# Hjinhan/Transgo

Measured on AMD Instinct MI355X. Metric: MCTS simulations/sec, higher is better.
Workload: dtype f32

## Files before the change

### include/transgo_hip.h

```cpp
#ifndef TRANSGO_HIP_H_
#define TRANSGO_HIP_H_

#include <stdbool.h>
#include <stddef.h>
#include <stdint.h>

#ifdef __cplusplus
extern "C" {
#endif

typedef struct tg_ctx tg_ctx;

typedef enum tg_status {
    TG_OK = 0,
    TG_ERR_ARG = -1,
    TG_ERR_HIP = -2,
    TG_ERR_NO_DEVICE = -3,
    TG_ERR_ARENA = -4,
    TG_ERR_STATE = -5
} tg_status;

typedef struct tg_config {
    int32_t board_size;
    int32_t encode_dim;
// ... 56 lines not shown

int tg_sp_collect(tg_ctx* ctx, int32_t* n_active, int32_t* n_rows);
int tg_sp_absorb(tg_ctx* ctx);
int tg_sp_search(tg_ctx* ctx, int32_t* n_waves);

int tg_sp_root_info(tg_ctx* ctx, int32_t* visits , int32_t* root_n, int32_t* player, int32_t* step,
                    float* obs );
int tg_sp_draw_uniform(tg_ctx* ctx, double* u , const uint8_t* mask);
int tg_sp_rng_state(tg_ctx* ctx, int game, tg_mt19937* out);
int tg_sp_rng_get(tg_ctx* ctx, tg_mt19937* out );
int tg_sp_rng_set(tg_ctx* ctx, const tg_mt19937* in , const uint8_t* mask );
int tg_sp_play(tg_ctx* ctx, const int32_t* actions , uint8_t* done );
int tg_sp_game_errors(tg_ctx* ctx, int32_t* n_errors, int32_t* err );
int tg_sp_tree_truncations(tg_ctx* ctx, uint64_t* blocks);

int tg_sp_pool_stats(tg_ctx* ctx, uint64_t* pool_slots, uint64_t* high_water_slots, uint64_t* in_use_slots, uint64_t* exhausted);

int tg_sp_finished(tg_ctx* ctx, int32_t* n_games, int32_t* n_positions);
int tg_sp_harvest(tg_ctx* ctx, uint32_t* obs_bits, int32_t* counts, float* z, int8_t* own, uint8_t* player, int device_out,
                  int32_t* slot, int32_t* n_moves, int32_t* winner, float* score, int8_t* terr);
int tg_sp_final(tg_ctx* ctx, float* score , float* terr , int32_t* winner );
int tg_sp_stats(tg_ctx* ctx, uint64_t* sims, uint64_t* evals, uint64_t* depth_sum, uint64_t* tie_draws, int32_t* errors,
                int32_t* max_slots);

size_t tg_net_blob_floats(int board_size, int encode_dim, int filters, int blocks);
int tg_net_load(tg_ctx* ctx, const float* blob, size_t n_floats, int rows_cap);
size_t tg_net_blob_floats_arch(int board_size, int encode_dim, int filters, const char* arch);
int tg_net_load_arch(tg_ctx* ctx, const char* arch, const float* blob, size_t n_floats, int rows_cap);
int tg_net_load_async(tg_ctx* ctx, const char* arch, const float* blob, size_t n_floats);
int tg_net_load_async_dev(tg_ctx* ctx, const char* arch, const float* d_blob , size_t n_floats);
int tg_net_load_poll(tg_ctx* ctx, int wait, int* pending);
int tg_net_predict(tg_ctx* ctx, const float* obs, int n_rows, float* policy, float* value, float* own);
int tg_net_range(tg_ctx* ctx, uint64_t* fp16_overflows, float* weight_absmax);
int tg_prof_enable(tg_ctx* ctx, int on, int max_launches);
int tg_prof_read(tg_ctx* ctx, double* conv_ms, int64_t* conv_launches, double* conv_flops);
int tg_prof_skipped(tg_ctx* ctx, int64_t* launches);
int tg_prof_enable_tree(tg_ctx* ctx, int on, int max_waves);
int tg_prof_read_tree(tg_ctx* ctx, double* collect_ms, double* absorb_ms, int64_t* waves, uint64_t* children_scored);

typedef struct tg_replay tg_replay;
int tg_replay_create(tg_ctx* ctx, int capacity_positions, tg_replay** out);
void tg_replay_destroy(tg_replay* rp);
int tg_replay_append(tg_replay* rp, const uint32_t* obs_bits , const int32_t* counts ,
                     const float* z , const int8_t* own , int n);
int tg_replay_append_dev(tg_replay* rp, const uint32_t* obs_bits, const int32_t* counts, const float* z, const int8_t* own, int n);
int tg_replay_info(const tg_replay* rp, long long* entries, long long* index, int* full);
int tg_replay_sample(tg_replay* rp, const long long* entry , int B, float* state , float* pi ,
                     float* z , float* own , int device_out);


void tg_host_mt_seed(tg_mt19937* s, uint32_t seed);
uint32_t tg_host_mt_next32(tg_mt19937* s);
double tg_host_mt_random_sample(tg_mt19937* s);
int32_t tg_host_mt_choice_index(tg_mt19937* s, int32_t k);
int tg_host_mt_dirichlet(tg_mt19937* s, double alpha, int32_t n, double* out);
void tg_host_sub_encode(int board_size, const void* encode, void* sub_encode, int sub_board_size, int channels, int cut_num);


#ifndef TRANSGO_NO_GOENV_NAMES
bool Init(int history_dim, int encode_dim, int max_step, float komi);
bool Reset(void* state);
bool Step(const void* state, void* next_state, int16_t action);
bool Step_(void* state, int16_t action);
bool checkAction(const void* state, int16_t action);
bool isTerminated(const void* state);
bool Encode(const void* state, float* encode_state);
// ... 15 lines not shown
```

### transgo_amd/_lib.py

```python
import ctypes
import os

_HERE = os.path.dirname(os.path.abspath(__file__))
LIB_PATH = os.path.join(_HERE, "libtransgo_hip.so")


class TgConfig(ctypes.Structure):
    _fields_ = [("board_size", ctypes.c_int32), ("encode_dim", ctypes.c_int32), ("max_step", ctypes.c_int32),
                ("komi", ctypes.c_float), ("n_games", ctypes.c_int32), ("num_simulation", ctypes.c_int32),
                ("parallel_readouts", ctypes.c_int32), ("wu_loss", ctypes.c_int32), ("c_puct1", ctypes.c_double),
                ("c_puct2", ctypes.c_double), ("arena_slots", ctypes.c_int32), ("net_blocks", ctypes.c_int32),
                ("net_filters", ctypes.c_int32), ("device", ctypes.c_int32), ("net_precision", ctypes.c_int32),
                ("record_games", ctypes.c_int32), ("pool_slots", ctypes.c_int32), ("reserved", ctypes.c_int32 * 5)]


class TgMt19937(ctypes.Structure):
    _fields_ = [("key", ctypes.c_uint32 * 624), ("pos", ctypes.c_int32)]


class TransgoError(RuntimeError):
    pass


_lib = None
# ... 15 lines not shown
    "tg_sp_reset_from": (ctypes.c_int, [_vp, _vp, _vp]),
    "tg_sp_root_states": (ctypes.c_int, [_vp, _vp]),
    "tg_sp_batch_rows": (ctypes.c_int, [_vp, ctypes.POINTER(ctypes.c_int32)]),
    "tg_sp_batch_obs": (ctypes.c_int, [_vp, _vp, ctypes.c_int32]),
    "tg_sp_set_eval": (ctypes.c_int, [_vp, _vp, _vp, ctypes.c_int32]),
    "tg_sp_eval": (ctypes.c_int, [_vp]),
    "tg_sp_expand_roots": (ctypes.c_int, [_vp]),
    "tg_sp_begin_move": (ctypes.c_int, [_vp, ctypes.c_int, ctypes.c_int]),
    "tg_sp_collect": (ctypes.c_int, [_vp, ctypes.POINTER(ctypes.c_int32), ctypes.POINTER(ctypes.c_int32)]),
    "tg_sp_absorb": (ctypes.c_int, [_vp]),
    "tg_sp_search": (ctypes.c_int, [_vp, ctypes.POINTER(ctypes.c_int32)]),
    "tg_sp_root_info": (ctypes.c_int, [_vp, _vp, _vp, _vp, _vp, _vp]),
    "tg_sp_draw_uniform": (ctypes.c_int, [_vp, _vp, _vp]),
    "tg_sp_rng_state": (ctypes.c_int, [_vp, ctypes.c_int, ctypes.POINTER(TgMt19937)]),
    "tg_sp_rng_get": (ctypes.c_int, [_vp, _vp]),
    "tg_sp_rng_set": (ctypes.c_int, [_vp, _vp, _vp]),
    "tg_sp_play": (ctypes.c_int, [_vp, _vp, _vp]),
    "tg_sp_final": (ctypes.c_int, [_vp, _vp, _vp, _vp]),
    "tg_sp_game_errors": (ctypes.c_int, [_vp, ctypes.POINTER(ctypes.c_int32), _vp]),
    "tg_sp_tree_truncations": (ctypes.c_int, [_vp, ctypes.POINTER(ctypes.c_uint64)]),
    "tg_sp_pool_stats": (ctypes.c_int, [_vp] + [ctypes.POINTER(ctypes.c_uint64)] * 4),
    "tg_sp_finished": (ctypes.c_int, [_vp, ctypes.POINTER(ctypes.c_int32), ctypes.POINTER(ctypes.c_int32)]),
    "tg_sp_harvest": (ctypes.c_int, [_vp, _vp, _vp, _vp, _vp, _vp, ctypes.c_int, _vp, _vp, _vp, _vp, _vp]),
    "tg_sp_stats": (ctypes.c_int, [_vp] + [ctypes.POINTER(ctypes.c_uint64)] * 4 + [ctypes.POINTER(ctypes.c_int32)] * 2),
    "tg_net_blob_floats": (ctypes.c_size_t, [ctypes.c_int] * 4),
    "tg_net_load": (ctypes.c_int, [_vp, _vp, ctypes.c_size_t, ctypes.c_int]),
    "tg_net_blob_floats_arch": (ctypes.c_size_t, [ctypes.c_int] * 3 + [ctypes.c_char_p]),
    "tg_net_load_arch": (ctypes.c_int, [_vp, ctypes.c_char_p, _vp, ctypes.c_size_t, ctypes.c_int]),
    "tg_net_load_async": (ctypes.c_int, [_vp, ctypes.c_char_p, _vp, ctypes.c_size_t]),
    "tg_net_load_async_dev": (ctypes.c_int, [_vp, ctypes.c_char_p, _vp, ctypes.c_size_t]),
    "tg_net_load_poll": (ctypes.c_int, [_vp, ctypes.c_int, ctypes.POINTER(ctypes.c_int)]),
    "tg_net_predict": (ctypes.c_int, [_vp, _vp, ctypes.c_int, _vp, _vp, _vp]),
    "tg_net_range": (ctypes.c_int, [_vp, ctypes.POINTER(ctypes.c_uint64), ctypes.POINTER(ctypes.c_float)]),
    "tg_prof_enable": (ctypes.c_int, [_vp, ctypes.c_int, ctypes.c_int]),
    "tg_prof_read": (ctypes.c_int, [_vp, ctypes.POINTER(ctypes.c_double), ctypes.POINTER(ctypes.c_int64), ctypes.POINTER(ctypes.c_double)]),
    "tg_prof_skipped": (ctypes.c_int, [_vp, ctypes.POINTER(ctypes.c_int64)]),
    "tg_prof_enable_tree": (ctypes.c_int, [_vp, ctypes.c_int, ctypes.c_int]),
    "tg_prof_read_tree": (ctypes.c_int, [_vp, ctypes.POINTER(ctypes.c_double), ctypes.POINTER(ctypes.c_double), ctypes.POINTER(ctypes.c_int64),
                                          ctypes.POINTER(ctypes.c_uint64)]),
    "tg_replay_create": (ctypes.c_int, [_vp, ctypes.c_int, ctypes.POINTER(ctypes.c_void_p)]),
    "tg_replay_destroy": (None, [_vp]),
    "tg_replay_append": (ctypes.c_int, [_vp, _vp, _vp, _vp, _vp, ctypes.c_int]),
    "tg_replay_append_dev": (ctypes.c_int, [_vp, _vp, _vp, _vp, _vp, ctypes.c_int]),
    "tg_replay_info": (ctypes.c_int, [_vp, ctypes.POINTER(ctypes.c_longlong), ctypes.POINTER(ctypes.c_longlong), ctypes.POINTER(ctypes.c_int)]),
    "tg_replay_sample": (ctypes.c_int, [_vp, _vp, ctypes.c_int, _vp, _vp, _vp, _vp, ctypes.c_int]),
    "tg_host_mt_seed": (None, [ctypes.POINTER(TgMt19937), ctypes.c_uint32]),
    "tg_host_mt_next32": (ctypes.c_uint32, [ctypes.POINTER(TgMt19937)]),
    "tg_host_mt_random_sample": (ctypes.c_double, [ctypes.POINTER(TgMt19937)]),
    "tg_host_mt_choice_index": (ctypes.c_int32, [ctypes.POINTER(TgMt19937), ctypes.c_int32]),
    "tg_host_sub_encode": (None, [ctypes.c_int, _vp, _vp, ctypes.c_int, ctypes.c_int, ctypes.c_int]),
    "tg_host_mt_dirichlet": (ctypes.c_int, [ctypes.POINTER(TgMt19937), ctypes.c_double, ctypes.c_int32, _vp]),
}


def load():
    global _lib
    if _lib is not None:
        return _lib
    try:
        import torch
    except ImportError:
        pass
    if not os.path.exists(LIB_PATH):
        raise TransgoError(f"{LIB_PATH} not found: build it with `make -C transgo_amd/csrc` "
                           "(or python -c 'import __graft_entry__ as g; g.build()'); there is no CPU fallback")
    lib = ctypes.CDLL(LIB_PATH)
# ... 47 lines not shown
```

### transgo_amd/csrc/conv_rows.h

```cpp
#pragma once

namespace tg {

constexpr int conv_sg_rows(int boards, int P) { return ((boards + 15) >> 4) * 16 * P; }
constexpr int conv_sg_row(int b, int p, int P) { return ((b >> 4) * P + p) * 16 + (b & 15); }

constexpr unsigned conv_tap_mask(int p, int S) {
    const int x = p % S, y = p / S;
    unsigned mk = 0;
    for (int tap = 0; tap < 9; ++tap) {
        const int yy = y + tap / 3 - 1, xx = x + tap % 3 - 1;
        if (yy >= 0 && yy < S && xx >= 0 && xx < S) mk |= 1u << tap;
    }
    return mk;
}
constexpr int conv_tap_count(unsigned mask) {
    int n = 0;
    for (int tap = 0; tap < 9; ++tap) n += (mask >> tap) & 1;
    return n;
}
constexpr unsigned long long conv_tap_list(unsigned mask) {
    unsigned long long l = 0;
    int k = 0;
    for (int tap = 0; tap < 9; ++tap)
        if ((mask >> tap) & 1) { l |= (unsigned long long)tap << (4 * k); ++k; }
    return l;
}

constexpr int conv_pos_of(int idx, int S) {
    const int I = S - 2;
    if (idx < I * I) return (1 + idx / I) * S + 1 + idx % I;
    const int e = idx - I * I;
    if (e < 4 * I) {
        const int side = e / I, k = 1 + e % I;
        return side == 0 ? k : side == 1 ? (S - 1) * S + k : side == 2 ? k * S : k * S + S - 1;
    }
    const int c = e - 4 * I;
    return (c >> 1) * (S - 1) * S + (c & 1) * (S - 1);
}

}
```

### transgo_amd/csrc/net.hip

```cpp
#include <cmath>
#include <cstdlib>
#include <cstring>
#include <string>
#include <vector>

#include "conv_rows.h"
#include "engine.h"

using namespace tg;

namespace tg {

struct ConvW { const float* w; const float* b; };
struct BlockW { const float* s1; const float* t1; ConvW c1; ConvW c2; const float* g1; const float* g2;
                const _Float16* h1; const _Float16* h2; };
struct AttW { ConvW qkv; const float* gamma; const float* s; const float* t;
              const _Float16* x3w = nullptr; const float* x3sc = nullptr; };
struct Layer { int kind; int ridx; AttW a; };

enum Chain { CHAIN_F32 = 0, CHAIN_DMA, CHAIN_F16, CHAIN_SPLIT };
struct NetPath {
    Chain chain = CHAIN_F32;
    bool r16 = false;
    bool att_x3 = false;
// ... 3 lines not shown

struct Net {
    int F = 0, NB = 0, C = 0, S = 0, P = 0, A = 0;
    float* blob = nullptr; size_t blob_floats = 0;
    float* wstage = nullptr;
    ConvW stem; std::vector<BlockW> blocks; std::vector<Layer> layers; const float* s_end = nullptr; const float* t_end = nullptr;
    bool pol_att = false; AttW patt; ConvW head_a; std::string arch;
    float* bufQ = nullptr; float* hca = nullptr;
    float* bufAct = nullptr;
    int prec = 0;
    const float* head_g = nullptr; const float* head_ag = nullptr;
    const _Float16* head_x2 = nullptr; const float* head_x2sc = nullptr;
    float* wsc = nullptr;
    _Float16* stem_h = nullptr; _Float16* head_h = nullptr; _Float16* x0h = nullptr;
    _Float16* wh = nullptr; _Float16* act16 = nullptr; _Float16* h16 = nullptr;
    NetPath path;
    ConvW head; const float* w_vo = nullptr; const float* b_vo = nullptr; const float* w_v = nullptr; const float* b_v = nullptr;
    const float* w_o = nullptr; const float* b_o = nullptr; const float* w_a = nullptr; const float* b_a = nullptr;
    const uint32_t* in_bits = nullptr; const int32_t* in_slot = nullptr; int in_words = 0;
    float* x0 = nullptr;
    float* bufA = nullptr; float* bufB = nullptr; float* bufH = nullptr;
    float* hc = nullptr;
    float* own = nullptr;
    int rows_cap = 0;
    unsigned* range = nullptr;
    struct WeightSet { float* blob = nullptr; float* wstage = nullptr; _Float16* wh = nullptr; _Float16* stem_h = nullptr; _Float16* head_h = nullptr;
                       float* wsc = nullptr; float* head_g = nullptr; float* head_ag = nullptr;
                       _Float16* att_h = nullptr; float* att_sc = nullptr;
                       _Float16* head_x2 = nullptr; float* head_x2sc = nullptr; };
    WeightSet sets[2]; int active = 0; bool pending = false;
    hipStream_t side = nullptr; hipEvent_t loaded = nullptr, swapped = nullptr; float* pinned = nullptr;
    bool prof = false; std::vector<hipEvent_t> ev; size_t ev_used = 0; double conv_ms = 0; long conv_launches = 0; double conv_flops = 0;
    long conv_skipped = 0;
};

}

namespace {

using f32x4 = __attribute__((ext_vector_type(4))) float;
using f32x2 = __attribute__((ext_vector_type(2))) float;
using h2 = __attribute__((ext_vector_type(2))) _Float16;
using h8 = __attribute__((ext_vector_type(8))) _Float16;
using h4 = __attribute__((ext_vector_type(4))) _Float16;
__device__ __forceinline__ int tid0() { return (int)threadIdx.x; }



template <int S>
__global__ __launch_bounds__(256) void k_obs_to_rows(const float* __restrict__ obs, float* __restrict__ x0, int rows, int C) {
    constexpr int P = S * S;
    const size_t total = (size_t)rows * P * 16;
    for (size_t i = (size_t)blockIdx.x * 256 + threadIdx.x; i < total; i += (size_t)gridDim.x * 256) {
        const int c = (int)(i & 15);
        const size_t m = i >> 4;
        const int p = (int)(m % P);
        const size_t r = m / P;
        x0[i] = c < C ? obs[(r * C + c) * P + p] : 0.f;
    }
}


template <int S>
__global__ __launch_bounds__(256) void k_bits_to_rows(const uint32_t* __restrict__ bits, const int32_t* __restrict__ row_slot,
                                                      float* __restrict__ x0, int rows, int C, int W) {
    constexpr int P = S * S;
// ... 186 lines not shown
                }
            }
        }
    }
    int mrow[NPT], srow[NPT];
#pragma unroll
    for (int t = 0; t < NPT; ++t) {
        mrow[t] = m0 + (wave * NPT + t) * 16 + j;
        srow[t] = SM2 ? conv_sg_row(mrow[t] / P, mrow[t] % P, P) : mrow[t];
    }
    conv_epilogue<COUT, CT, NPT, EPI, false, SM2>(acc, mrow, M, 0, kq, out, res, out2, par, srow, conv_sg_rows(M / P, P));
}

typedef __attribute__((address_space(3))) void tg_lds_void;
#define TG_VMCNT(N) asm volatile("s_waitcnt vmcnt(%0)" ::"n"(N) : "memory")
#define TG_BARRIER() do { asm volatile("" ::: "memory"); __builtin_amdgcn_s_barrier(); asm volatile("" ::: "memory"); } while (0)

using u32x4 = __attribute__((ext_vector_type(4))) unsigned int;
__device__ __forceinline__ u32x4 tg_rsrc(const void* base, unsigned bytes) {
    const unsigned long long a = (unsigned long long)base;
    return u32x4{(unsigned)a, (unsigned)(a >> 32) & 0xffffu, bytes, 0x00020000u};
}
__device__ __forceinline__ void tg_dma_global(const void* sbase , int voff_bytes, tg_lds_void* lds) {
    const unsigned la = __builtin_amdgcn_readfirstlane((unsigned)(unsigned long long)lds);
    asm volatile("s_mov_b32 m0, %0\n\ts_nop 0\n\tglobal_load_lds_dwordx4 %1, %2" ::"s"(la), "v"(voff_bytes), "s"(sbase) : "memory");
}
__device__ __forceinline__ void tg_dma_buffer(u32x4 rsrc, int voff_bytes, tg_lds_void* lds) {
    const unsigned la = __builtin_amdgcn_readfirstlane((unsigned)(unsigned long long)lds);
    asm volatile("s_mov_b32 m0, %0\n\ts_nop 0\n\tbuffer_load_dwordx4 %1, %2, 0 offen lds" ::"s"(la), "v"(voff_bytes), "s"(rsrc) : "memory");
}

__device__ __forceinline__ int swz64(int row) { return ((row >> 2) & 1) << 1; }

template <int S, int F, int EPI>
__global__ __launch_bounds__(256, (F == 128 ? 4 : 2)) void k_conv3x3_sg(const float* __restrict__ in, float* __restrict__ out,
                                                                       const float* __restrict__ res, const float* __restrict__ Ws,
                                                                       const float* __restrict__ bias, float* __restrict__ out2,
                                                                       const float* __restrict__ s2, const float* __restrict__ t2, int rows) {
    constexpr int P = S * S, CT = F / 16, CC = 16;
    constexpr int NPT = 2, TB = 64 * NPT;
    constexpr int WPW = CT / 4;
    constexpr int NSL = F / CC, D = 4;
    static_assert((F == 128 || F == 256) && NSL % 2 == 0, "tile geometry");
    __shared__ __attribute__((aligned(16))) float ws[D][F * CC];
    __shared__ __attribute__((aligned(16))) float par[3 * F];
    const int tid = threadIdx.x, lane = tid & 63;
    const int wave = __builtin_amdgcn_readfirstlane(tid >> 6);
    const int j = lane & 15, kq = lane >> 4;
    const int tpx = ((int)gridDim.x + 7) >> 3;
    const int bid = ((int)blockIdx.x & 7) * tpx + ((int)blockIdx.x >> 3);
    const int nrange = (rows + TB - 1) / TB;
    if (bid >= nrange * P) return;
    const int range = bid / P;
    const int p = conv_pos_of(bid - range * P, S);
    const int M = rows * P, Msm = conv_sg_rows(rows, P);
    for (int i = tid; i < F; i += 256) { par[i] = bias[i]; par[F + i] = out2 ? s2[i] : 0.f; par[2 * F + i] = out2 ? t2[i] : 0.f; }

    const unsigned mask = conv_tap_mask(p, S);
    const int nt = conv_tap_count(mask), nst = NSL * nt;
    const unsigned long long taps = conv_tap_list(mask);
    const int inv = nt == 9 ? 7282 : nt == 6 ? 10923 : 16384;
    auto stage = [&](int k, int* sl, int* tap) {
        *sl = (k * inv) >> 16;
        *tap = (int)(taps >> (4 * (k - *sl * nt))) & 15;
    };

    const __amdgpu_buffer_rsrc_t rin = __builtin_amdgcn_make_buffer_rsrc(const_cast<float*>(in), 0, Msm * F * 4, 0x00020000);
    const int prow = lane >> 2, pchunk = (lane & 3) ^ swz64(lane >> 2);
    auto dma_w = [&](int k) {
        int sl, tap;
        stage(k, &sl, &tap);
        const float* src = Ws + (size_t)(sl * 9 + tap) * (F * CC);
#pragma unroll
        for (int i = 0; i < WPW; ++i) {
            const int pc = wave * WPW + i;
            tg_dma_global(src + pc * 16 * CC, (prow * CC + pchunk * 4) * 4, (tg_lds_void*)(&ws[k & (D - 1)][pc * 256]));
        }
    };
    const int aoff = j * CC + ((kq ^ swz64(j)) << 2);
    const int grp0 = (range * 4 + wave) * NPT;
    const bool active = grp0 * 16 < rows;
    const int boff = ((conv_sg_row(grp0 * 16 + j, p, P)) * CC + kq * 4) * 4;
    f32x4 acc[CT][NPT], b_cur[NPT], b_next[NPT];
    auto load_b = [&](f32x4* b, int k) {
        int sl, tap;
        stage(k, &sl, &tap);
        const int ty = (tap * 11) >> 5;
        const int soff = (sl * Msm + ((ty - 1) * S + (tap - 3 * ty - 1)) * 16) * (CC * 4);
#pragma unroll
        for (int t = 0; t < NPT; ++t)
            b[t] = __builtin_bit_cast(f32x4, __builtin_amdgcn_raw_buffer_load_b128(rin, (int)((unsigned)boff + (unsigned)soff + (unsigned)(t * (P * 16 * CC * 4))), 0, 0));
    };
#pragma unroll
    for (int k = 0; k < D; ++k) dma_w(k);
    if (active) {
#pragma unroll
        for (int t = 0; t < NPT; ++t) {
            const int b = (grp0 + t) * 16 + j;
            const int m = b < rows ? b * P + p : M - 1;
#pragma unroll
            for (int ct = 0; ct < CT; ++ct) {
                acc[ct][t] = f32x4{0.f, 0.f, 0.f, 0.f};
                if (EPI == 1) acc[ct][t] = *reinterpret_cast<const f32x4*>(res + (size_t)m * F + ct * 16 + kq * 4);
            }
        }
        load_b(b_cur, 0);
        TG_VMCNT((EPI == 1 ? CT * NPT : 0) + NPT);
    } else {
        TG_VMCNT(0);
    }
    asm volatile("s_waitcnt lgkmcnt(0)" ::: "memory");
    TG_BARRIER();

#pragma unroll 1
    for (int k0 = 0; k0 < nst; k0 += 2) {
#pragma unroll
        for (int h = 0; h < 2; ++h) {
            const int k = k0 + h;
            if (active) {
                const float* wcur = ws[k & (D - 1)];
                if (k + 1 < nst) load_b(b_next, k + 1);
                __builtin_amdgcn_sched_barrier(0);
                f32x4 a_cur = *reinterpret_cast<const f32x4*>(wcur + aoff);
#pragma unroll
                for (int ct = 0; ct < CT; ++ct) {
                    f32x4 a_next = a_cur;
                    if (ct + 1 < CT) a_next = *reinterpret_cast<const f32x4*>(wcur + (ct + 1) * 256 + aoff);
#pragma unroll
                    for (int s4 = 0; s4 < 4; ++s4)
#pragma unroll
                        for (int t = 0; t < NPT; ++t)
                            acc[ct][t] = __builtin_amdgcn_mfma_f32_16x16x4f32(a_cur[s4], b_cur[t][s4], acc[ct][t], 0, 0, 0);
                    a_cur = a_next;
                }
#pragma unroll
                for (int t = 0; t < NPT; ++t) b_cur[t] = b_next[t];
            }
            TG_VMCNT(0);
        }
        TG_BARRIER();
        if (k0 + 4 < nst) { dma_w(k0 + 4); dma_w(k0 + 5); }
    }
    if (!active) return;
    int mrow[NPT], srow[NPT];
#pragma unroll
    for (int t = 0; t < NPT; ++t) {
        const int b = (grp0 + t) * 16 + j;
        mrow[t] = b < rows ? b * P + p : M;
        srow[t] = conv_sg_row(b, p, P);
    }
    conv_epilogue<F, CT, NPT, (EPI == 1 ? 2 : EPI), EPI == 0, true>(acc, mrow, M, 0, kq, out, res, out2, par, srow, Msm);
}

__device__ __forceinline__ size_t h16_index(int m, int c, int M) { return (((size_t)(c >> 5) * 4 + ((c >> 3) & 3)) * M + m) * 8 + (c & 7); }

template <int N>
__device__ __forceinline__ void vmcnt_uniform(int n) {
    if (n >= N) TG_VMCNT(N);
    else if constexpr (N > 0) vmcnt_uniform<N - 1>(n);
}

__device__ __forceinline__ int x2_index(int c) { return ((c >> 4) << 5) + (c & 15); }
template <int F, int CT, int NPT, int EPI, bool R16, bool X2 = false>
__device__ __forceinline__ void conv_epilogue_h8(f32x4 (&acc)[CT][NPT], const int (&mrow)[NPT], int M, int co_base, int kq,
                                                 float* __restrict__ out32, _Float16* __restrict__ out16, const float* par, int pstride,
                                                 float wsc, float& amax) {
    static_assert(CT % 2 == 0, "tile pairs");
    static_assert(!(X2 && R16), "split precision keeps the f32 residual stream");
#pragma unroll
    for (int t = 0; t < NPT; ++t) {
        if (mrow[t] >= M) continue;
#pragma unroll
        for (int u = 0; u < CT / 2; ++u) {
            const int lc = u * 32 + kq * 8, col = co_base + lc;
            f32x4 v[2];
#pragma unroll
            for (int h = 0; h < 2; ++h) v[h] = (X2 ? acc[2 * u + h][t] * wsc : acc[2 * u + h][t]) + *reinterpret_cast<const f32x4*>(par + lc + 4 * h);
            h8 o;
            if constexpr (X2) {
                auto store_split = [&](const f32x4 (&w)[2]) {
                    h8 hi, lo;
#pragma unroll
                    for (int e = 0; e < 8; ++e) { const float x = w[e >> 2][e & 3]; hi[e] = (_Float16)x; lo[e] = (_Float16)(x - (float)hi[e]); }
#pragma unroll
// ... 1241 lines not shown
    }
    if (own)
        for (int o = tid; o < P; o += 256) {
            float a[HR];
#pragma unroll
            for (int r = 0; r < HR; ++r) a[r] = b_o[o];
            for (int k = 0; k < 64; ++k) {
                const float w = w_o[k * P + o];
#pragma unroll
                for (int r = 0; r < HR; ++r) a[r] = fmaf(hid[r][k], w, a[r]);
            }
#pragma unroll
            for (int r = 0; r < HR; ++r) if (r < nr) own[(size_t)(row0 + r) * P + o] = tanhf(a[r]);
        }
    __syncthreads();
    for (int i = tid; i < HR * A; i += 256) { const int r = i / A, o = i % A; logit[r][o] = expf(logit[r][o] - red[r][0]); }
    __syncthreads();
    if (tid < nr) { float s2 = 0.f; for (int o = 0; o < A; ++o) s2 += logit[tid][o]; red[tid][1] = s2; }
    __syncthreads();
    for (int i = tid; i < nr * A; i += 256) {
        const int r = i / A, o = i % A;
        policy[(size_t)(row0 + r) * A + o] = logit[r][o] * (1.f / red[r][1]);
    }
}

struct ProfScope {
    Net* n; hipStream_t st; bool on;
    ProfScope(Net* net, hipStream_t s, double flops) : n(net), st(s), on(net->prof && net->ev_used + 2 <= net->ev.size()) {
        if (on) { (void)hipEventRecord(n->ev[n->ev_used], st); n->conv_flops += flops; n->conv_launches++; }
        else if (net->prof) n->conv_skipped++;
    }
    ~ProfScope() { if (on) { (void)hipEventRecord(n->ev[n->ev_used + 1], st); n->ev_used += 2; } }
};

template <int S, int F>
int forward_t(tg_ctx* ctx, Net* n, const float* obs, int rows, float* policy, float* value, float* own) {
    constexpr int P = S * S;
    constexpr bool WIDE = F == 128 || F == 256;
    hipStream_t st = ctx->stream;
    const int M = rows * P;
    const int grid = (M + 127) / 128;
    constexpr int NPT = F <= 128 ? 3 : 2;
    const int grid_f = (M + 64 * NPT - 1) / (64 * NPT);
    const int grid_h = (M + 255) / 256;
    constexpr int COS = F / 128;
    const int nblk_h2 = COS == 1 ? grid_h : (grid_h + 7) / 8 * 8 * COS;
    const double conv_flops = 2.0 * 9.0 * (double)F * (double)F * (double)M;
    constexpr int WQ = F / 4 + F / 4 + F;
    const bool big = (long long)M * F * 4 >= (1ll << 31);
    Chain chain = n->path.chain;
    if (chain == CHAIN_DMA && (long long)conv_sg_rows(rows, P) * F * 4 >= (1ll << 31)) chain = CHAIN_F32;
    if (chain == CHAIN_SPLIT && big) TG_FAIL(ctx, TG_ERR_ARG, "split-precision path: rows * P * F * 4 bytes must stay below 2 GiB per activation buffer");
    if (chain == CHAIN_F16 && (long long)M * F * 2 >= (1ll << 31)) TG_FAIL(ctx, TG_ERR_ARG, "fp16 path: rows * P * F * 2 bytes must stay below 2 GiB per activation buffer");
    const bool h16 = chain == CHAIN_F16 || chain == CHAIN_SPLIT, x2 = chain == CHAIN_SPLIT;
    const bool head16 = chain == CHAIN_F16 || (x2 && n->path.head_x2);
    auto wsc = [&](size_t conv) { return x2 ? n->wsc + conv : nullptr; };
    const size_t nl = n->layers.size(), nb = n->blocks.size();
    auto next_bn = [&](size_t j, const float** sn, const float** tn) -> bool {
        *sn = nullptr; *tn = nullptr;
        if (chain == CHAIN_F32) return false;
        if (j < nl && n->layers[j].kind == 0) { const BlockW& b = n->blocks[n->layers[j].ridx]; *sn = b.s1; *tn = b.t1; return true; }
        if (j == nl && head16) { *sn = n->s_end; *tn = n->t_end; return true; }
        return false;
    };

    float* x = n->bufA; float* y = n->bufB;
    auto stem = [&](bool act, const float* sn, const float* tn) {
        if constexpr (WIDE) {
            if (h16) {
                auto* k = x2 ? &k_conv3x3_h2<S, 64, F, 4, false, true> : n->path.r16 ? &k_conv3x3_h2<S, 64, F, 4, true> : &k_conv3x3_h2<S, 64, F, 4>;
                hipLaunchKernelGGL(k, dim3(nblk_h2), dim3(256), 0, st, n->x0h, x, act ? n->act16 : nullptr, nullptr, n->stem_h, n->stem.b,
                                   sn, tn, M, nblk_h2, wsc(2 * nb), n->range);
                return;
            }
            if (chain == CHAIN_DMA) {
                hipLaunchKernelGGL((k_conv3x3<S, 16, F, false, 0, 9, 2, true>), dim3(grid), dim3(256), 0, st, n->x0, x, nullptr, n->stem.w,
                                   n->stem.b, nullptr, nullptr, M, act ? n->bufAct : nullptr, sn, tn);
                return;
            }
        }
        hipLaunchKernelGGL((k_conv3x3<S, 16, F, false, 0>), dim3(grid), dim3(256), 0, st, n->x0, x, nullptr, n->stem.w, n->stem.b, nullptr, nullptr, M);
    };
    auto block = [&](const BlockW& b, int ridx, float* out, bool act, const float* sn, const float* tn) {
        if constexpr (WIDE) {
            if (h16) {
                auto* k1 = x2 ? &k_conv3x3_h2<S, 2 * F, F, 0, false, true> : &k_conv3x3_h2<S, F, F, 0>;
                auto* k2 = x2 ? &k_conv3x3_h2<S, 2 * F, F, 1, false, true> : n->path.r16 ? &k_conv3x3_h2<S, F, F, 1, true> : &k_conv3x3_h2<S, F, F, 1>;
                { ProfScope ps(n, st, conv_flops);
                  hipLaunchKernelGGL(k1, dim3(nblk_h2), dim3(256), 0, st, n->act16, nullptr, n->h16, nullptr, b.h1, b.c1.b, nullptr, nullptr,
                                     M, nblk_h2, wsc(2 * ridx), n->range); }
                { ProfScope ps(n, st, conv_flops);
                  hipLaunchKernelGGL(k2, dim3(nblk_h2), dim3(256), 0, st, n->h16, out, act ? n->act16 : nullptr, x, b.h2, b.c2.b, sn, tn,
                                     M, nblk_h2, wsc(2 * ridx + 1), n->range); }
                return;
            }
            if (chain == CHAIN_DMA) {
                const int grid_sd = ((rows + 127) / 128 * P + 7) / 8 * 8;
                auto* k1 = &k_conv3x3_sg<S, F, 0>;
                auto* k2 = &k_conv3x3_sg<S, F, 1>;
                { ProfScope ps(n, st, conv_flops);
                  hipLaunchKernelGGL(k1, dim3(grid_sd), dim3(256), 0, st, n->bufAct, n->bufH, nullptr, b.g1, b.c1.b, nullptr, nullptr, nullptr, rows); }
                { ProfScope ps(n, st, conv_flops);
                  hipLaunchKernelGGL(k2, dim3(grid_sd), dim3(256), 0, st, n->bufH, out, x, b.g2, b.c2.b, act ? n->bufAct : nullptr, sn, tn, rows); }
                return;
            }
        }
        { ProfScope ps(n, st, conv_flops);
          hipLaunchKernelGGL((k_conv3x3<S, F, F, true, 0, 9, NPT>), dim3(grid_f), dim3(256), 0, st, x, n->bufH, nullptr, b.c1.w, b.c1.b, b.s1, b.t1, M); }
        { ProfScope ps(n, st, conv_flops);
          hipLaunchKernelGGL((k_conv3x3<S, F, F, false, 1, 9, NPT>), dim3(grid_f), dim3(256), 0, st, n->bufH, out, x, b.c2.w, b.c2.b, nullptr, nullptr, M); }
    };
    auto attention = [&](const AttW& a, const float* xin, float* xout, const float* ps, const float* pt, bool act, const float* sn, const float* tn) -> int {
        if constexpr (S == 9 && F == 128) {
            if (x2) {
                constexpr int lds3 = (int)(sizeof(_Float16) * F / 16 * WQ * 32 + sizeof(float) * (WQ + 6 * F) + 4096);
                const int nwg = (rows + 3) / 4 < 256 ? (rows + 3) / 4 : 256;
                auto* k = ps ? &k_attention_x3<S, F, true> : &k_attention_x3<S, F, false>;
                hipLaunchKernelGGL(k, dim3(nwg), dim3(256), lds3, st, xin, xout, act ? n->act16 : nullptr, a.x3w, a.qkv.b, a.x3sc,
                                   a.gamma, a.s, a.t, ps, pt, sn, tn, rows, n->range);
                return 0;
            }
        }
        if (chain == CHAIN_F32 && !n->path.att_lds) return -1;
        auto* kq = ps ? &k_conv3x3<S, F, WQ, true, 2, 1> : &k_conv3x3<S, F, WQ, false, 2, 1>;
        hipLaunchKernelGGL(kq, dim3(grid), dim3(256), 0, st, xin, n->bufQ, nullptr, a.qkv.w, a.qkv.b, ps, pt, M, nullptr, nullptr, nullptr);
        if constexpr (S == 9 && F == 256) {
            if (x2) {
                hipLaunchKernelGGL((k_attention_mfma<S, F, 2, true>), dim3((rows + 3) / 4), dim3(256), 0, st, n->bufQ, xin, xout,
                                   reinterpret_cast<float*>(act ? n->act16 : nullptr), a.gamma, a.s, a.t, ps, pt, sn, tn, rows, n->range);
                return 0;
            }
        }
        if constexpr (S == 9 && WIDE) {
            if (chain == CHAIN_DMA) {
                hipLaunchKernelGGL((k_attention_mfma<S, F, 2>), dim3((rows + 3) / 4), dim3(256), 0, st, n->bufQ, xin, xout,
                                   act ? n->bufAct : nullptr, a.gamma, a.s, a.t, ps, pt, sn, tn, rows);
// ... 473 lines not shown
        ctx->err = "fp16 overflow: " + std::to_string(host[0]) + " epilogue tiles rounded a value beyond +-65504 to fp16 (net_precision " +
                   std::to_string(n->prec) + "); outputs since then may be inf/NaN -- use net_precision 0 for these weights";
    return TG_OK;
}

int tg_prof_enable(tg_ctx* ctx, int on, int max_launches) {
    if (!ctx || !ctx->eng || !ctx->eng->net) return TG_ERR_STATE;
    Net* n = ctx->eng->net;
    TG_HIP(ctx, hipSetDevice(ctx->cfg.device));
    if (on) {
        const size_t want = 2 * (size_t)(max_launches > 0 ? max_launches : 4096);
        while (n->ev.size() < want) { hipEvent_t ev; TG_HIP(ctx, hipEventCreate(&ev)); n->ev.push_back(ev); }
        n->ev_used = 0; n->conv_ms = 0; n->conv_launches = 0; n->conv_flops = 0; n->conv_skipped = 0;
    }
    n->prof = on != 0;
    return TG_OK;
}

int tg_prof_read(tg_ctx* ctx, double* conv_ms, int64_t* conv_launches, double* conv_flops) {
    if (!ctx || !ctx->eng || !ctx->eng->net) return TG_ERR_STATE;
    Net* n = ctx->eng->net;
    TG_HIP(ctx, hipStreamSynchronize(ctx->stream));
    double ms = 0;
    for (size_t i = 0; i + 1 < n->ev_used; i += 2) {
        float t = 0; TG_HIP(ctx, hipEventElapsedTime(&t, n->ev[i], n->ev[i + 1])); ms += t;
    }
    n->conv_ms += ms; n->ev_used = 0;
    if (conv_ms) *conv_ms = n->conv_ms;
    if (conv_launches) *conv_launches = n->conv_launches;
    if (conv_flops) *conv_flops = n->conv_flops;
    return TG_OK;
}

int tg_prof_skipped(tg_ctx* ctx, int64_t* launches) {
    if (!ctx || !ctx->eng || !ctx->eng->net) return TG_ERR_STATE;
    if (launches) *launches = ctx->eng->net->conv_skipped;
    return TG_OK;
}

}
```

Before: 536,100.

## Make sg conv kernel persistent with tap-weighted per-XCD tile scheduling

Turns the k_conv3x3_sg convolution from one workgroup per tile into a persistent grid sized by an occupancy query. Each XCD gets a contiguous span of tiles balanced by tap count (interior 9, edge 6, corner 4), and a workgroup walks its tiles in serpentine order. While finishing one tile it prefetches the next tile's weights and inputs, aiming to cut launch and tail imbalance and to keep the DMA ring busy across tiles. In exchange it adds per-tile index arithmetic and a serialised loop, and relies on the occupancy query being accurate. It also adds optional timestamp instrumentation and a query API for the slot count.

```diff
diff --git a/include/transgo_hip.h b/include/transgo_hip.h
--- a/include/transgo_hip.h
+++ b/include/transgo_hip.h
@@ -112,6 +112,7 @@
 int tg_net_load_poll(tg_ctx* ctx, int wait, int* pending);
 int tg_net_predict(tg_ctx* ctx, const float* obs, int n_rows, float* policy, float* value, float* own);
 int tg_net_range(tg_ctx* ctx, uint64_t* fp16_overflows, float* weight_absmax);
+int tg_net_conv_slots(tg_ctx* ctx, int* slots);
 int tg_prof_enable(tg_ctx* ctx, int on, int max_launches);
 int tg_prof_read(tg_ctx* ctx, double* conv_ms, int64_t* conv_launches, double* conv_flops);
 int tg_prof_skipped(tg_ctx* ctx, int64_t* launches);
diff --git a/transgo_amd/_lib.py b/transgo_amd/_lib.py
--- a/transgo_amd/_lib.py
+++ b/transgo_amd/_lib.py
@@ -71,6 +71,7 @@
     "tg_net_load_poll": (ctypes.c_int, [_vp, ctypes.c_int, ctypes.POINTER(ctypes.c_int)]),
     "tg_net_predict": (ctypes.c_int, [_vp, _vp, ctypes.c_int, _vp, _vp, _vp]),
     "tg_net_range": (ctypes.c_int, [_vp, ctypes.POINTER(ctypes.c_uint64), ctypes.POINTER(ctypes.c_float)]),
+    "tg_net_conv_slots": (ctypes.c_int, [_vp, ctypes.POINTER(ctypes.c_int)]),
     "tg_prof_enable": (ctypes.c_int, [_vp, ctypes.c_int, ctypes.c_int]),
     "tg_prof_read": (ctypes.c_int, [_vp, ctypes.POINTER(ctypes.c_double), ctypes.POINTER(ctypes.c_int64), ctypes.POINTER(ctypes.c_double)]),
     "tg_prof_skipped": (ctypes.c_int, [_vp, ctypes.POINTER(ctypes.c_int64)]),
diff --git a/transgo_amd/csrc/conv_rows.h b/transgo_amd/csrc/conv_rows.h
--- a/transgo_amd/csrc/conv_rows.h
+++ b/transgo_amd/csrc/conv_rows.h
@@ -39,4 +39,48 @@
     return (c >> 1) * (S - 1) * S + (c & 1) * (S - 1);
 }
 
+constexpr int conv_class_begin(int c, int S) {
+    const int I = S - 2;
+    return c == 0 ? 0 : c == 1 ? I * I : c == 2 ? I * I + 4 * I : S * S;
 }
+constexpr int conv_class_taps(int c) { return c == 0 ? 9 : c == 1 ? 6 : 4; }
+constexpr int conv_range_taps(int S) { return (3 * S - 2) * (3 * S - 2); }
+constexpr int conv_class_before(int t, int c, int S) {
+    const int P = S * S, c0 = conv_class_begin(c, S), len = conv_class_begin(c + 1, S) - c0;
+    const int i = t % P - c0;
+    return (t / P) * len + (i < 0 ? 0 : i > len ? len : i);
+}
+constexpr long long conv_taps_before(int t, int S) {
+    long long sum = 0;
+    for (int c = 0; c < 3; ++c) sum += (long long)conv_class_before(t, c, S) * conv_class_taps(c);
+    return sum;
+}
+constexpr int conv_xcd_begin(int x, int ntiles, int spx, int S) {
+    if (ntiles <= 8 * spx) return (int)((long long)x * ntiles / 8);
+    const int P = S * S, SP = conv_range_taps(S);
+    const long long target = (x * conv_taps_before(ntiles, S) + 7) / 8;
+    int rem = (int)(target % SP), i = 0;
+    for (int c = 0; c < 3 && rem > 0; ++c) {
+        const int len = conv_class_begin(c + 1, S) - conv_class_begin(c, S), nt = conv_class_taps(c);
+        if (rem >= len * nt) { rem -= len * nt; i += len; }
+        else { i += (rem + nt - 1) / nt; rem = 0; }
+    }
+    return (int)(target / SP) * P + i;
+}
+constexpr int conv_xcd_tile(int i, int t0, int t1, int S) {
+    for (int c = 0; c < 3; ++c) {
+        const int c0 = conv_class_begin(c, S), len = conv_class_begin(c + 1, S) - c0;
+        const int first = conv_class_before(t0, c, S), n = conv_class_before(t1, c, S) - first;
+        if (i < n) { const int g = first + i; return (g / len) * (S * S) + c0 + g % len; }
+        i -= n;
+    }
+    return -1;
+}
+constexpr int conv_slot_count(int s, int spx, int n) {
+    const int full = n / spx, rem = n % spx;
+    return full + ((full & 1) ? spx - 1 - s < rem : s < rem);
+}
+constexpr int conv_slot_index(int s, int k, int spx) { return k * spx + ((k & 1) ? spx - 1 - s : s); }
+constexpr int conv_slots_per_xcd(int slots, int ntiles) { const int g = slots < ntiles ? slots : ntiles; return (g + 7) / 8; }
+
+}
diff --git a/transgo_amd/csrc/net.hip b/transgo_amd/csrc/net.hip
--- a/transgo_amd/csrc/net.hip
+++ b/transgo_amd/csrc/net.hip
@@ -59,6 +59,7 @@
     hipStream_t side = nullptr; hipEvent_t loaded = nullptr, swapped = nullptr; float* pinned = nullptr;
     bool prof = false; std::vector<hipEvent_t> ev; size_t ev_used = 0; double conv_ms = 0; long conv_launches = 0; double conv_flops = 0;
     long conv_skipped = 0;
+    int conv_slots = 0;
 };
 
 }
@@ -311,44 +312,64 @@
 
 __device__ __forceinline__ int swz64(int row) { return ((row >> 2) & 1) << 1; }
 
+#ifdef TG_CONV_STAMP
+constexpr int TG_CONV_STAMP_CAP = 16384;
+__device__ unsigned long long tg_conv_stamps[2][TG_CONV_STAMP_CAP][8];
+#define TG_CSTAMP(tile, what, value) do { if (threadIdx.x == 0 && (tile) < TG_CONV_STAMP_CAP) tg_conv_stamps[EPI][tile][what] = (value); } while (0)
+#else
+#define TG_CSTAMP(tile, what, value) do { } while (0)
+#endif
 template <int S, int F, int EPI>
 __global__ __launch_bounds__(256, (F == 128 ? 4 : 2)) void k_conv3x3_sg(const float* __restrict__ in, float* __restrict__ out,
                                                                        const float* __restrict__ res, const float* __restrict__ Ws,
                                                                        const float* __restrict__ bias, float* __restrict__ out2,
-                                                                       const float* __restrict__ s2, const float* __restrict__ t2, int rows) {
+                                                                       const float* __restrict__ s2, const float* __restrict__ t2, int rows,
+                                                                       int spx) {
     constexpr int P = S * S, CT = F / 16, CC = 16;
     constexpr int NPT = 2, TB = 64 * NPT;
     constexpr int WPW = CT / 4;
     constexpr int NSL = F / CC, D = 4;
-    static_assert((F == 128 || F == 256) && NSL % 2 == 0, "tile geometry");
+    static_assert((F == 128 || F == 256) && NSL % D == 0, "tile geometry; every walk a multiple of the ring");
     __shared__ __attribute__((aligned(16))) float ws[D][F * CC];
     __shared__ __attribute__((aligned(16))) float par[3 * F];
     const int tid = threadIdx.x, lane = tid & 63;
     const int wave = __builtin_amdgcn_readfirstlane(tid >> 6);
     const int j = lane & 15, kq = lane >> 4;
-    const int tpx = ((int)gridDim.x + 7) >> 3;
-    const int bid = ((int)blockIdx.x & 7) * tpx + ((int)blockIdx.x >> 3);
-    const int nrange = (rows + TB - 1) / TB;
-    if (bid >= nrange * P) return;
-    const int range = bid / P;
-    const int p = conv_pos_of(bid - range * P, S);
+    const int ntiles = (rows + TB - 1) / TB * P;
+    const int xg = (int)blockIdx.x & 7, slot = (int)blockIdx.x >> 3;
+    const int t0 = conv_xcd_begin(xg, ntiles, spx, S), t1 = conv_xcd_begin(xg + 1, ntiles, spx, S);
+    const int nk = conv_slot_count(slot, spx, t1 - t0);
+    if (nk == 0) return;
+#ifdef TG_CONV_STAMP
+    unsigned long long stamp0 = __builtin_amdgcn_s_memtime();
+#endif
     const int M = rows * P, Msm = conv_sg_rows(rows, P);
     for (int i = tid; i < F; i += 256) { par[i] = bias[i]; par[F + i] = out2 ? s2[i] : 0.f; par[2 * F + i] = out2 ? t2[i] : 0.f; }
 
-    const unsigned mask = conv_tap_mask(p, S);
-    const int nt = conv_tap_count(mask), nst = NSL * nt;
-    const unsigned long long taps = conv_tap_list(mask);
-    const int inv = nt == 9 ? 7282 : nt == 6 ? 10923 : 16384;
-    auto stage = [&](int k, int* sl, int* tap) {
-        *sl = (k * inv) >> 16;
-        *tap = (int)(taps >> (4 * (k - *sl * nt))) & 15;
+    struct Tile { int id, p, nt, inv, grp0; unsigned long long taps; bool active; };
+    auto tile_at = [&](int k) {
+        Tile T;
+        T.id = conv_xcd_tile(conv_slot_index(slot, k, spx), t0, t1, S);
+        const int range = T.id / P;
+        T.p = conv_pos_of(T.id - range * P, S);
+        const unsigned mask = conv_tap_mask(T.p, S);
+        T.nt = conv_tap_count(mask);
+        T.taps = conv_tap_list(mask);
+        T.inv = T.nt == 9 ? 7282 : T.nt == 6 ? 10923 : 16384;
+        T.grp0 = (range * 4 + wave) * NPT;
+        T.active = T.grp0 * 16 < rows;
+        return T;
+    };
+    auto stage = [&](const Tile& T, int k, int* sl, int* tap) {
+        *sl = (k * T.inv) >> 16;
+        *tap = (int)(T.taps >> (4 * (k - *sl * T.nt))) & 15;
     };
 
     const __amdgpu_buffer_rsrc_t rin = __builtin_amdgcn_make_buffer_rsrc(const_cast<float*>(in), 0, Msm * F * 4, 0x00020000);
     const int prow = lane >> 2, pchunk = (lane & 3) ^ swz64(lane >> 2);
-    auto dma_w = [&](int k) {
+    auto dma_w = [&](const Tile& T, int k) {
         int sl, tap;
-        stage(k, &sl, &tap);
+        stage(T, k, &sl, &tap);
         const float* src = Ws + (size_t)(sl * 9 + tap) * (F * CC);
 #pragma unroll
         for (int i = 0; i < WPW; ++i) {
@@ -357,78 +378,118 @@
         }
     };
     const int aoff = j * CC + ((kq ^ swz64(j)) << 2);
-    const int grp0 = (range * 4 + wave) * NPT;
-    const bool active = grp0 * 16 < rows;
-    const int boff = ((conv_sg_row(grp0 * 16 + j, p, P)) * CC + kq * 4) * 4;
+    const int boff = (j * CC + kq * 4) * 4;
     f32x4 acc[CT][NPT], b_cur[NPT], b_next[NPT];
-    auto load_b = [&](f32x4* b, int k) {
+#pragma unroll
+    for (int t = 0; t < NPT; ++t) b_cur[t] = b_next[t] = f32x4{0.f, 0.f, 0.f, 0.f};
+    auto load_b = [&](f32x4* b, const Tile& T, int k) {
         int sl, tap;
-        stage(k, &sl, &tap);
+        stage(T, k, &sl, &tap);
         const int ty = (tap * 11) >> 5;
-        const int soff = (sl * Msm + ((ty - 1) * S + (tap - 3 * ty - 1)) * 16) * (CC * 4);
+        const int soff = (sl * Msm + (T.grp0 * P + T.p + (ty - 1) * S + (tap - 3 * ty - 1)) * 16) * (CC * 4);
 #pragma unroll
         for (int t = 0; t < NPT; ++t)
             b[t] = __builtin_bit_cast(f32x4, __builtin_amdgcn_raw_buffer_load_b128(rin, (int)((unsigned)boff + (unsigned)soff + (unsigned)(t * (P * 16 * CC * 4))), 0, 0));
     };
-#pragma unroll
-    for (int k = 0; k < D; ++k) dma_w(k);
-    if (active) {
+    auto init_acc = [&](const Tile& T) {
+        int m[NPT];
 #pragma unroll
         for (int t = 0; t < NPT; ++t) {
-            const int b = (grp0 + t) * 16 + j;
-            const int m = b < rows ? b * P + p : M - 1;
-#pragma unroll
-            for (int ct = 0; ct < CT; ++ct) {
+            const int b = (T.grp0 + t) * 16 + j;
+            m[t] = b < rows ? b * P + T.p : M - 1;
+        }
+#pragma unroll
+        for (int ct = 0; ct < CT; ++ct)
+#pragma unroll
+            for (int t = 0; t < NPT; ++t) {
                 acc[ct][t] = f32x4{0.f, 0.f, 0.f, 0.f};
-                if (EPI == 1) acc[ct][t] = *reinterpret_cast<const f32x4*>(res + (size_t)m * F + ct * 16 + kq * 4);
-            }
-        }
-        load_b(b_cur, 0);
+                if (EPI == 1) acc[ct][t] = *reinterpret_cast<const f32x4*>(res + (size_t)m[t] * F + ct * 16 + kq * 4);
+            }
+    };
+
+    Tile cur = tile_at(0);
+#pragma unroll
+    for (int k = 0; k < D; ++k) dma_w(cur, k);
+    if (cur.active) {
+        init_acc(cur);
+        load_b(b_cur, cur, 0);
         TG_VMCNT((EPI == 1 ? CT * NPT : 0) + NPT);
     } else {
         TG_VMCNT(0);
     }
     asm volatile("s_waitcnt lgkmcnt(0)" ::: "memory");
     TG_BARRIER();
+#ifdef TG_CONV_STAMP
+    TG_CSTAMP(cur.id, 7, __builtin_amdgcn_s_memrealtime());
+    unsigned long long stamp1 = __builtin_amdgcn_s_memtime();
+#endif
 
 #pragma unroll 1
-    for (int k0 = 0; k0 < nst; k0 += 2) {
-#pragma unroll
-        for (int h = 0; h < 2; ++h) {
-            const int k = k0 + h;
-            if (active) {
-                const float* wcur = ws[k & (D - 1)];
-                if (k + 1 < nst) load_b(b_next, k + 1);
+    for (int ti = 0;; ++ti) {
+        const bool more = ti + 1 < nk;
+        Tile nxt = cur;
+        if (more) nxt = tile_at(ti + 1);
+        const int nst = NSL * cur.nt;
+#pragma unroll 1
+        for (int k0 = 0; k0 < nst; k0 += 2) {
+#pragma unroll
+            for (int h = 0; h < 2; ++h) {
+                const int k = k0 + h;
+                if (k + 1 < nst) { if (cur.active) load_b(b_next, cur, k + 1); }
+                else if (more && nxt.active) load_b(b_next, nxt, 0);
                 __builtin_amdgcn_sched_barrier(0);
-                f32x4 a_cur = *reinterpret_cast<const f32x4*>(wcur + aoff);
-#pragma unroll
-                for (int ct = 0; ct < CT; ++ct) {
-                    f32x4 a_next = a_cur;
-                    if (ct + 1 < CT) a_next = *reinterpret_cast<const f32x4*>(wcur + (ct + 1) * 256 + aoff);
-#pragma unroll
-                    for (int s4 = 0; s4 < 4; ++s4)
-#pragma unroll
-                        for (int t = 0; t < NPT; ++t)
-                            acc[ct][t] = __builtin_amdgcn_mfma_f32_16x16x4f32(a_cur[s4], b_cur[t][s4], acc[ct][t], 0, 0, 0);
-                    a_cur = a_next;
+                if (cur.active) {
+                    const float* wcur = ws[k & (D - 1)];
+                    f32x4 a_cur = *reinterpret_cast<const f32x4*>(wcur + aoff);
+#pragma unroll
+                    for (int ct = 0; ct < CT; ++ct) {
+                        f32x4 a_next = a_cur;
+                        if (ct + 1 < CT) a_next = *reinterpret_cast<const f32x4*>(wcur + (ct + 1) * 256 + aoff);
+#pragma unroll
+                        for (int s4 = 0; s4 < 4; ++s4)
+#pragma unroll
+                            for (int t = 0; t < NPT; ++t)
+                                acc[ct][t] = __builtin_amdgcn_mfma_f32_16x16x4f32(a_cur[s4], b_cur[t][s4], acc[ct][t], 0, 0, 0);
+                        a_cur = a_next;
+                    }
                 }
 #pragma unroll
                 for (int t = 0; t < NPT; ++t) b_cur[t] = b_next[t];
-            }
-            TG_VMCNT(0);
-        }
-        TG_BARRIER();
-        if (k0 + 4 < nst) { dma_w(k0 + 4); dma_w(k0 + 5); }
-    }
-    if (!active) return;
-    int mrow[NPT], srow[NPT];
-#pragma unroll
-    for (int t = 0; t < NPT; ++t) {
-        const int b = (grp0 + t) * 16 + j;
-        mrow[t] = b < rows ? b * P + p : M;
-        srow[t] = conv_sg_row(b, p, P);
-    }
-    conv_epilogue<F, CT, NPT, (EPI == 1 ? 2 : EPI), EPI == 0, true>(acc, mrow, M, 0, kq, out, res, out2, par, srow, Msm);
+                TG_VMCNT(0);
+            }
+            TG_BARRIER();
+            if (k0 + 4 < nst) { dma_w(cur, k0 + 4); dma_w(cur, k0 + 5); }
+            else if (more) { dma_w(nxt, k0 + 4 - nst); dma_w(nxt, k0 + 5 - nst); }
+        }
+#ifdef TG_CONV_STAMP
+        const unsigned long long stamp2 = __builtin_amdgcn_s_memtime();
+#endif
+        if (cur.active) {
+            int mrow[NPT], srow[NPT];
+#pragma unroll
+            for (int t = 0; t < NPT; ++t) {
+                const int b = (cur.grp0 + t) * 16 + j;
+                mrow[t] = b < rows ? b * P + cur.p : M;
+                srow[t] = conv_sg_row(b, cur.p, P);
+            }
+            conv_epilogue<F, CT, NPT, (EPI == 1 ? 2 : EPI), EPI == 0, true>(acc, mrow, M, 0, kq, out, res, out2, par, srow, Msm);
+        }
+#ifdef TG_CONV_STAMP
+        {
+            const unsigned long long stamp3 = __builtin_amdgcn_s_memtime();
+            TG_CSTAMP(cur.id, 0, stamp0); TG_CSTAMP(cur.id, 1, stamp1); TG_CSTAMP(cur.id, 2, stamp2); TG_CSTAMP(cur.id, 3, stamp3);
+            TG_CSTAMP(cur.id, 5, (unsigned long long)(__builtin_amdgcn_s_getreg((3 << 11) | 20) & 15) | (unsigned long long)nst << 8 |
+                                 (unsigned long long)ti << 20 | (unsigned long long)blockIdx.x << 32);
+            TG_CSTAMP(cur.id, 6, (unsigned long long)__builtin_amdgcn_s_getreg((31 << 11) | 4));
+            if (ti > 0) TG_CSTAMP(cur.id, 7, 0ull);
+            if (!more) { TG_VMCNT(0); TG_CSTAMP(cur.id, 4, __builtin_amdgcn_s_memtime()); } else TG_CSTAMP(cur.id, 4, 0ull);
+            stamp0 = stamp1 = stamp3;
+        }
+#endif
+        if (!more) break;
+        cur = nxt;
+        if (cur.active) init_acc(cur);
+    }
 }
 
 __device__ __forceinline__ size_t h16_index(int m, int c, int M) { return (((size_t)(c >> 5) * 4 + ((c >> 3) & 3)) * M + m) * 8 + (c & 7); }
@@ -1736,6 +1797,22 @@
     }
     ~ProfScope() { if (on) { (void)hipEventRecord(n->ev[n->ev_used + 1], st); n->ev_used += 2; } }
 };
+
+template <int S, int F>
+int conv_sg_slots(int device) {
+#ifdef TG_CONV_ONE_TILE
+    return 1 << 28;
+#endif
+    int cus = 0, nb0 = 0, nb1 = 0;
+    if (hipDeviceGetAttribute(&cus, hipDeviceAttributeMultiprocessorCount, device) != hipSuccess) return -1;
+    if (hipOccupancyMaxActiveBlocksPerMultiprocessor(&nb0, k_conv3x3_sg<S, F, 0>, 256, 0) != hipSuccess) return -1;
+    if (hipOccupancyMaxActiveBlocksPerMultiprocessor(&nb1, k_conv3x3_sg<S, F, 1>, 256, 0) != hipSuccess) return -1;
+    const int cap = F == 128 ? 4 : 2;
+    int nb = nb0 < nb1 ? nb0 : nb1;
+    nb = nb < 1 ? 1 : nb > cap ? cap : nb;
+    const int slots = cus * nb / 8 * 8;
+    return slots < 8 ? 8 : slots;
+}
 
 template <int S, int F>
 int forward_t(tg_ctx* ctx, Net* n, const float* obs, int rows, float* policy, float* value, float* own) {
@@ -1768,6 +1845,13 @@
         return false;
     };
 
+    if constexpr (WIDE) {
+        if (chain == CHAIN_DMA) {
+            if (!n->conv_slots) n->conv_slots = conv_sg_slots<S, F>(ctx->cfg.device);
+            if (n->conv_slots <= 0) TG_FAIL(ctx, TG_ERR_HIP, "occupancy query of k_conv3x3_sg failed");
+        }
+    }
+
     float* x = n->bufA; float* y = n->bufB;
     auto stem = [&](bool act, const float* sn, const float* tn) {
         if constexpr (WIDE) {
@@ -1799,13 +1883,13 @@
                 return;
             }
             if (chain == CHAIN_DMA) {
-                const int grid_sd = ((rows + 127) / 128 * P + 7) / 8 * 8;
+                const int spx = conv_slots_per_xcd(n->conv_slots, (rows + 127) / 128 * P), grid_sd = 8 * spx;
                 auto* k1 = &k_conv3x3_sg<S, F, 0>;
                 auto* k2 = &k_conv3x3_sg<S, F, 1>;
                 { ProfScope ps(n, st, conv_flops);
-                  hipLaunchKernelGGL(k1, dim3(grid_sd), dim3(256), 0, st, n->bufAct, n->bufH, nullptr, b.g1, b.c1.b, nullptr, nullptr, nullptr, rows); }
+                  hipLaunchKernelGGL(k1, dim3(grid_sd), dim3(256), 0, st, n->bufAct, n->bufH, nullptr, b.g1, b.c1.b, nullptr, nullptr, nullptr, rows, spx); }
                 { ProfScope ps(n, st, conv_flops);
-                  hipLaunchKernelGGL(k2, dim3(grid_sd), dim3(256), 0, st, n->bufH, out, x, b.g2, b.c2.b, act ? n->bufAct : nullptr, sn, tn, rows); }
+                  hipLaunchKernelGGL(k2, dim3(grid_sd), dim3(256), 0, st, n->bufH, out, x, b.g2, b.c2.b, act ? n->bufAct : nullptr, sn, tn, rows, spx); }
                 return;
             }
         }
@@ -2345,6 +2429,29 @@
     return TG_OK;
 }
 
+int tg_net_conv_slots(tg_ctx* ctx, int* slots) {
+    if (!ctx || !ctx->eng || !ctx->eng->net || !slots) return TG_ERR_STATE;
+    Net* n = ctx->eng->net;
+    TG_HIP(ctx, hipSetDevice(ctx->cfg.device));
+    *slots = 0;
+    if (n->path.chain != CHAIN_DMA) return TG_OK;
+    if (!n->conv_slots) {
+        if (n->S == 9 && n->F == 128) n->conv_slots = conv_sg_slots<9, 128>(ctx->cfg.device);
+        if (n->S == 9 && n->F == 256) n->conv_slots = conv_sg_slots<9, 256>(ctx->cfg.device);
+        if (n->S == 19 && n->F == 128) n->conv_slots = conv_sg_slots<19, 128>(ctx->cfg.device);
+        if (n->S == 19 && n->F == 256) n->conv_slots = conv_sg_slots<19, 256>(ctx->cfg.device);
+    }
+    if (n->conv_slots < 0) TG_FAIL(ctx, TG_ERR_HIP, "occupancy query of k_conv3x3_sg failed");
+    *slots = n->conv_slots;
+    return TG_OK;
+}
+
+#ifdef TG_CONV_STAMP
+int tg_debug_conv_stamps(void* out) {
+    return hipMemcpyFromSymbol(out, HIP_SYMBOL(tg_conv_stamps), sizeof(tg_conv_stamps)) == hipSuccess ? 0 : 1;
+}
+#endif
+
 int tg_prof_skipped(tg_ctx* ctx, int64_t* launches) {
     if (!ctx || !ctx->eng || !ctx->eng->net) return TG_ERR_STATE;
     if (launches) *launches = ctx->eng->net->conv_skipped;
```

Result: slower. 512,600 (-4.4%).
